# LiZhuoHong/SegLand

Measured on AMD Instinct MI355X. Metric: 512x512 tiles/sec fwd+bwd PSPNet-POP, higher is better.
Workload: dtype bf16; 1 GPU; PSPNet-POP resnet50 bf16, batch 16/GPU, 512x512, 8 logit channels, train_base.py loop body (fwd+loss+bwd+clip+AdamW x2), 1 x MI355X; global_batch=16, parallelism=dp1

## Files before the change

### segland_amd/csrc/ppm.hip

```cpp
#include "common.h"

namespace {

struct PpmGeom {
  int B, H, W, C, nlevels;
  int sizes[4];
  int rowoff[5];
  int ncy, ncx;
  int yb[40], xb[40];
};

inline int bin_start(int i, int in, int out) { return (i * in) / out; }
inline int bin_end(int i, int in, int out) { return ((i + 1) * in + out - 1) / out; }
__device__ __forceinline__ int d_bin_start(int i, int in, int out) { return (i * in) / out; }
__device__ __forceinline__ int d_bin_end(int i, int in, int out) { return ((i + 1) * in + out - 1) / out; }

int make_bounds(const SlPpmDesc* d, int in, int* out) {
  bool mark[4097] = {false};
  if (in > 4096) return -1;
  for (int l = 0; l < d->nlevels; ++l)
    for (int i = 0; i < d->sizes[l]; ++i) { mark[bin_start(i, in, d->sizes[l])] = true; mark[bin_end(i, in, d->sizes[l])] = true; }
  int n = 0;
  for (int v = 0; v <= in; ++v) if (mark[v]) { if (n >= 40) return -1; out[n++] = v; }
  return n - 1;
}

int make_geom(const SlPpmDesc* d, PpmGeom& g) {
  SL_REQUIRE(d && d->B > 0 && d->H > 0 && d->W > 0 && d->C > 0 && d->C % 8 == 0, "ppm: bad sizes");
  SL_REQUIRE(d->nlevels >= 1 && d->nlevels <= 4, "ppm: 1..4 levels");
  g.B = d->B; g.H = d->H; g.W = d->W; g.C = d->C; g.nlevels = d->nlevels;
  int off = 0;
  for (int l = 0; l < 4; ++l) {
    g.sizes[l] = l < d->nlevels ? d->sizes[l] : 0;
    g.rowoff[l] = off;
    if (l < d->nlevels) { SL_REQUIRE(d->sizes[l] >= 1 && d->sizes[l] <= 64, "ppm: bad level size"); off += d->B * d->sizes[l] * d->sizes[l]; }
  }
  g.rowoff[4] = off;
  g.ncy = make_bounds(d, d->H, g.yb);
  g.ncx = make_bounds(d, d->W, g.xb);
  SL_REQUIRE(g.ncy > 0 && g.ncx > 0, "ppm: too many distinct bin boundaries");
  return 0;
}

template <typename T>
__global__ void ppm_cells_kernel(PpmGeom g, const T* __restrict__ x, float* __restrict__ cells) {
  constexpr int V = Vec16<T>::N;
  const int nv = g.C / V;
  const long long total = (long long)g.B * g.ncy * g.ncx * nv;
  for (long long i = blockIdx.x * (long long)blockDim.x + threadIdx.x; i < total; i += (long long)gridDim.x * blockDim.x) {
    const int v = (int)(i % nv); long long r = i / nv;
    const int cx = (int)(r % g.ncx); r /= g.ncx;
    const int cy = (int)(r % g.ncy); const int b = (int)(r / g.ncy);
    float s[V];
#pragma unroll
    for (int k = 0; k < V; ++k) s[k] = 0.f;
    for (int y = g.yb[cy]; y < g.yb[cy + 1]; ++y)
      for (int xx = g.xb[cx]; xx < g.xb[cx + 1]; ++xx) {
        float t[V];
        unpack16<T>(*(const uint4*)(x + ((size_t)(b * g.H + y) * g.W + xx) * g.C + v * V), t);
#pragma unroll
        for (int k = 0; k < V; ++k) s[k] += t[k];
      }
    float* o = cells + (size_t)i * V;
#pragma unroll
    for (int k = 0; k < V; ++k) o[k] = s[k];
  }
}

template <typename T>
__global__ __launch_bounds__(256) void ppm_cells_rows_kernel(PpmGeom g, const T* __restrict__ x, float* __restrict__ cells) {
  constexpr int V = Vec16<T>::N;
  __shared__ float red[8][32][V + 1];
  const int nv = g.C / V, vblocks = (nv + 31) / 32;
  int bid = blockIdx.x;
  const int vb = bid % vblocks; bid /= vblocks;
  const int cx = bid % g.ncx; bid /= g.ncx;
  const int cy = bid % g.ncy; const int b = bid / g.ncy;
  const int lv = threadIdx.x & 31, rl = threadIdx.x >> 5;
  const int v = vb * 32 + lv;
  float s[V];
#pragma unroll
  for (int k = 0; k < V; ++k) s[k] = 0.f;
  if (v < nv)
    for (int y = g.yb[cy] + rl; y < g.yb[cy + 1]; y += 8)
      for (int xx = g.xb[cx]; xx < g.xb[cx + 1]; ++xx) {
        float t[V];
        unpack16<T>(*(const uint4*)(x + ((size_t)(b * g.H + y) * g.W + xx) * g.C + v * V), t);
#pragma unroll
        for (int k = 0; k < V; ++k) s[k] += t[k];
      }
#pragma unroll
  for (int k = 0; k < V; ++k) red[rl][lv][k] = s[k];
  __syncthreads();
  if (rl == 0 && v < nv) {
    float* o = cells + ((((size_t)b * g.ncy + cy) * g.ncx + cx) * nv + v) * V;
#pragma unroll
    for (int k = 0; k < V; ++k) {
      float a = red[0][lv][k];
#pragma unroll
      for (int r = 1; r < 8; ++r) a += red[r][lv][k];
      o[k] = a;
    }
  }
}

__global__ void ppm_bins_kernel(PpmGeom g, const float* __restrict__ cells, float* __restrict__ pooled) {
  const long long total = (long long)g.rowoff[4] * g.C;
  for (long long i = blockIdx.x * (long long)blockDim.x + threadIdx.x; i < total; i += (long long)gridDim.x * blockDim.x) {
    const int c = (int)(i % g.C); const int row = (int)(i / g.C);
    int l = 0;
    while (l + 1 < g.nlevels && row >= g.rowoff[l + 1]) ++l;
    const int s = g.sizes[l];
    int r = row - g.rowoff[l];
    const int j = r % s; r /= s;
    const int ii = r % s; const int b = r / s;
    const int ys = d_bin_start(ii, g.H, s), ye = d_bin_end(ii, g.H, s), xs = d_bin_start(j, g.W, s), xe = d_bin_end(j, g.W, s);
    float sum = 0.f;
    for (int cy = 0; cy < g.ncy; ++cy) {
      if (g.yb[cy] < ys || g.yb[cy + 1] > ye) continue;
      for (int cx = 0; cx < g.ncx; ++cx) {
        if (g.xb[cx] < xs || g.xb[cx + 1] > xe) continue;
        sum += cells[(((size_t)b * g.ncy + cy) * g.ncx + cx) * g.C + c];
      }
    }
    pooled[i] = sum / (float)((ye - ys) * (xe - xs));
  }
}

__global__ void ppm_pool_bwd_cells_kernel(PpmGeom g, const float* __restrict__ dpooled, float* __restrict__ gcell) {
  const long long total = (long long)g.B * g.ncy * g.ncx * g.C;
  for (long long i = blockIdx.x * (long long)blockDim.x + threadIdx.x; i < total; i += (long long)gridDim.x * blockDim.x) {
    const int c = (int)(i % g.C); long long r = i / g.C;
    const int cx = (int)(r % g.ncx); r /= g.ncx;
    const int cy = (int)(r % g.ncy); const int b = (int)(r / g.ncy);
    const int y0 = g.yb[cy], y1 = g.yb[cy + 1], x0 = g.xb[cx], x1 = g.xb[cx + 1];
    float acc = 0.f;
    int nbins = 0;
    for (int l = 0; l < g.nlevels; ++l) nbins += g.sizes[l] * g.sizes[l];
    if (g.C % 64 == 0 && nbins <= 64) {
      const int lane = threadIdx.x & 63;
      float wq = 0.f; int rowq = 0;
      {
        int q = lane, l = 0;
        while (l < g.nlevels && q >= g.sizes[l] * g.sizes[l]) { q -= g.sizes[l] * g.sizes[l]; ++l; }
        if (l < g.nlevels) {
          const int s = g.sizes[l], ii = q / s, j = q - ii * s;
          const int ys = d_bin_start(ii, g.H, s), ye = d_bin_end(ii, g.H, s), xs = d_bin_start(j, g.W, s), xe = d_bin_end(j, g.W, s);
          if (!(y0 < ys || y1 > ye) && !(x0 < xs || x1 > xe)) { wq = 1.f / (float)((ye - ys) * (xe - xs)); rowq = g.rowoff[l] + (b * s + ii) * s + j; }
        }
      }
      for (int q = 0; q < nbins; ++q) {
        const float w = __shfl(wq, q, 64);
        if (w == 0.f) continue;
        acc += dpooled[(size_t)__shfl(rowq, q, 64) * g.C + c] * w;
      }
      gcell[i] = acc;
      continue;
    }
    for (int l = 0; l < g.nlevels; ++l) {
      const int s = g.sizes[l];
      for (int ii = 0; ii < s; ++ii) {
        const int ys = d_bin_start(ii, g.H, s), ye = d_bin_end(ii, g.H, s);
        if (y0 < ys || y1 > ye) continue;
        for (int j = 0; j < s; ++j) {
          const int xs = d_bin_start(j, g.W, s), xe = d_bin_end(j, g.W, s);
          if (x0 < xs || x1 > xe) continue;
          acc += dpooled[((size_t)g.rowoff[l] + (size_t)(b * s + ii) * s + j) * g.C + c] * (1.f / (float)((ye - ys) * (xe - xs)));
        }
      }
    }
    gcell[i] = acc;
  }
}

template <typename T>
__global__ __launch_bounds__(256) void ppm_pool_bwd_kernel(PpmGeom g, const float* __restrict__ gcell, const T* __restrict__ dcat, int cat_pitch, int cat_off,
                                                           T* __restrict__ dx) {
  constexpr int V = Vec16<T>::N;
  __shared__ int cxs[4096];
  const int by = blockIdx.x, b = by / g.H, y = by - b * g.H;
  int cy = 0;
  while (cy + 1 < g.ncy && y >= g.yb[cy + 1]) ++cy;
  for (int xx = threadIdx.x; xx < g.W; xx += 256) {
    int cx = 0;
    while (cx + 1 < g.ncx && xx >= g.xb[cx + 1]) ++cx;
    cxs[xx] = cx;
  }
  __syncthreads();
  const int nv = g.C / V;
  const float* gc = gcell + ((size_t)b * g.ncy + cy) * g.ncx * g.C;
  const size_t row = (size_t)by * g.W;
  for (int i = threadIdx.x; i < g.W * nv; i += 256) {
    const int xx = i / nv, v = i - xx * nv;
    float acc[V];
    if (dcat) unpack16<T>(*(const uint4*)(dcat + (row + xx) * cat_pitch + cat_off + v * V), acc);
    else {
#pragma unroll
      for (int k = 0; k < V; ++k) acc[k] = 0.f;
    }
    const float* t = gc + (size_t)cxs[xx] * g.C + v * V;
#pragma unroll
    for (int k = 0; k < V; k += 4) {
      const float4 q = *(const float4*)(t + k);
      acc[k] += q.x; acc[k + 1] += q.y; acc[k + 2] += q.z; acc[k + 3] += q.w;
    }
    *(uint4*)(dx + ((row + xx) * nv + v) * V) = pack16<T>(acc);
  }
}

__device__ __forceinline__ void src_index_ac0(int dst, int in, int out, int& i0, int& i1, float& l1) {
  const float scale = (float)in / (float)out;
  float src = scale * ((float)dst + 0.5f) - 0.5f;
  if (src < 0.f) src = 0.f;
  i0 = (int)src;
  i1 = i0 + (i0 < in - 1 ? 1 : 0);
  l1 = src - (float)i0;
  l1 = l1 < 0.f ? 0.f : (l1 > 1.f ? 1.f : l1);
}

template <typename T>
__global__ void ppm_upsample_fwd_kernel(PpmGeom g, int Cs, const float* __restrict__ stage, T* __restrict__ priors) {
  constexpr int V = Vec16<T>::N;
  const int nv = Cs / V, pitch = g.nlevels * Cs;
  const long long total = (long long)g.B * g.H * g.W * g.nlevels * nv;
  for (long long i = blockIdx.x * (long long)blockDim.x + threadIdx.x; i < total; i += (long long)gridDim.x * blockDim.x) {
    const int v = (int)(i % nv); long long r = i / nv;
    const int l = (int)(r % g.nlevels); r /= g.nlevels;
    const int xx = (int)(r % g.W); r /= g.W;
    const int y = (int)(r % g.H); const int b = (int)(r / g.H);
// ... 369 lines not shown
    SL_TRY(sl_launch("ppm_cells_rows_kernel", ppm_cells_rows_kernel<bf16_t>, dim3((unsigned)(g.B * g.ncy * g.ncx * ((g.C / 8 + 31) / 32))), dim3(256), 0, st, g, (const bf16_t*)x, cells));
  else
    SL_TRY(sl_by_dtype(d->dtype, "ppm_pool_fwd", [&](auto t) -> int {
      using T = decltype(t);
      return sl_launch("ppm_cells_kernel", ppm_cells_kernel<T>, dim3(gs_blocks((long long)g.B * g.ncy * g.ncx * g.C / Vec16<T>::N)), dim3(256), 0, st, g, (const T*)x, cells);
    }));
  return sl_launch("ppm_bins_kernel", ppm_bins_kernel, dim3(gs_blocks((long long)g.rowoff[4] * g.C)), dim3(256), 0, st, g, cells, pooled);
}

extern "C" int sl_ppm_pool_bwd(const SlPpmDesc* d, const float* dpooled, const void* dcat, int cat_pitch, int cat_off, void* dx,
                               void* workspace, size_t workspace_bytes, sl_stream_t stream) {
  PpmGeom g;
  if (int e = make_geom(d, g)) return e;
  SL_REQUIRE(dpooled && dx && workspace, "ppm_pool_bwd: null buffer");
  SL_REQUIRE(!dcat || (cat_pitch >= cat_off + g.C && cat_pitch % 8 == 0 && cat_off % 8 == 0), "ppm_pool_bwd: bad concat geometry");
  SL_REQUIRE(g.W <= 4096, "ppm_pool_bwd: W > 4096");
  const size_t need = (size_t)g.B * g.ncy * g.ncx * g.C * sizeof(float);
  if (workspace_bytes < need) { sl_set_error("ppm_pool_bwd: workspace %zu < %zu", workspace_bytes, need); return SL_EWORKSPACE; }
  hipStream_t st = (hipStream_t)stream;
  float* gcell = (float*)workspace;
  return sl_by_dtype(d->dtype, "ppm_pool_bwd", [&](auto t) -> int {
    using T = decltype(t);
    SL_TRY(sl_launch("ppm_pool_bwd_cells_kernel", ppm_pool_bwd_cells_kernel, dim3(gs_blocks((long long)g.B * g.ncy * g.ncx * g.C)), dim3(256), 0, st, g, dpooled, gcell));
    return sl_launch("ppm_pool_bwd_kernel", ppm_pool_bwd_kernel<T>, dim3(g.B * g.H), dim3(256), 0, st, g, gcell, (const T*)dcat, cat_pitch, cat_off, (T*)dx);
  });
}

extern "C" int sl_ppm_upsample_fwd(const SlPpmDesc* d, int Cs, const float* stage, void* priors, sl_stream_t stream) {
  PpmGeom g;
  if (int e = make_geom(d, g)) return e;
  SL_REQUIRE(stage && priors && Cs > 0 && Cs % 8 == 0, "ppm_upsample_fwd: bad args");
  return sl_by_dtype(d->dtype, "ppm_upsample_fwd", [&](auto t) -> int {
    using T = decltype(t);
    return sl_launch("ppm_upsample_fwd_kernel", ppm_upsample_fwd_kernel<T>, dim3(gs_blocks((long long)g.B * g.H * g.W * g.nlevels * Cs / Vec16<T>::N)), dim3(256), 0, (hipStream_t)stream, g, Cs, stage, (T*)priors);
  });
}

extern "C" int sl_ppm_upsample_bwd(const SlPpmDesc* d, int Cs, const void* dcat, int cat_pitch, float* dstage, void* workspace,
                                   size_t workspace_bytes, sl_stream_t stream) {
  PpmGeom g;
  if (int e = make_geom(d, g)) return e;
  SL_REQUIRE(dcat && dstage && workspace && Cs > 0 && Cs % 8 == 0 && cat_pitch >= g.nlevels * Cs, "ppm_upsample_bwd: bad args");
  const int nlj = sum_sizes(g);
  const size_t need = (size_t)g.B * g.H * nlj * Cs * sizeof(float);
  if (workspace_bytes < need) { sl_set_error("ppm_upsample_bwd: workspace %zu < %zu", workspace_bytes, need); return SL_EWORKSPACE; }
  hipStream_t st = (hipStream_t)stream;
  float* tmp = (float*)workspace;
// ... 339 lines not shown
```

### segland_amd/csrc/stem.hip

```cpp
#include "common.h"

namespace {

constexpr int TS = 16;
constexpr int PS = (TS - 1) * 2 + 7;
constexpr int NTAP = 147;

__device__ __forceinline__ void load_patch(float* patch, const float* img, int b, int H, int W, int oy0, int ox0, int tid) {
  for (int e = tid; e < 3 * PS * PS; e += 256) {
    const int c = e / (PS * PS), r = (e / PS) % PS, q = e % PS;
    const int iy = 2 * oy0 - 3 + r, ix = 2 * ox0 - 3 + q;
    float v = 0.f;
    if ((unsigned)iy < (unsigned)H && (unsigned)ix < (unsigned)W) v = img[((size_t)(b * 3 + c) * H + iy) * W + ix];
    patch[e] = v;
  }
}

template <typename T>
__global__ __launch_bounds__(256) void stem_conv_fwd_kernel(const float* __restrict__ img, const float* __restrict__ w,
                                                            T* __restrict__ y, float* __restrict__ part, int B, int H, int W) {
  extern __shared__ __attribute__((aligned(16))) float sm[];
  float* wl = sm;
  float* patch = sm + NTAP * 64;
  const int Ho = H / 2, Wo = W / 2;
// ... 54 lines not shown
      for (int k = 0; k < 16; ++k) {
        part[((size_t)blockIdx.x * 2 + 0) * 64 + cg * 16 + k] = s1[k];
        part[((size_t)blockIdx.x * 2 + 1) * 64 + cg * 16 + k] = s2[k];
      }
    }
  }
}

constexpr int MP = 38;
constexpr int KSTEPS = 10;

__global__ void stem_weight_frag_kernel(const float* __restrict__ w, uint4* __restrict__ wfrag) {
  const int t = blockIdx.x * blockDim.x + threadIdx.x;
  if (t >= 2 * KSTEPS * 64) return;
  const int lane = t & 63, ks = (t >> 6) % KSTEPS, nb = (t >> 6) / KSTEPS;
  const int n = nb * 32 + (lane & 31), k0 = ks * 16 + (lane >> 5) * 8;
  unsigned short v[8];
#pragma unroll
  for (int e = 0; e < 8; ++e) v[e] = k0 + e < NTAP ? from_f<bf16_t>(w[n * NTAP + k0 + e]) : (unsigned short)0;
  wfrag[t] = make_uint4(v[0] | ((unsigned)v[1] << 16), v[2] | ((unsigned)v[3] << 16), v[4] | ((unsigned)v[5] << 16), v[6] | ((unsigned)v[7] << 16));
}

__host__ __device__ constexpr int stem_tap_off(int k) { return k < NTAP ? ((k / 49) * PS + (k % 49) / 7) * MP + (k % 7) : 0; }

template <int KS>
__device__ __forceinline__ void stem_kstep(const bf16_t* __restrict__ patch, const int (&pbase)[2], int fh, const uint4* __restrict__ wfrag, int lane, f32x16_t (&acc)[2][2]) {
  const uint4 w0 = wfrag[(0 * KSTEPS + KS) * 64 + lane], w1 = wfrag[(1 * KSTEPS + KS) * 64 + lane];
  int off[8];
#pragma unroll
  for (int e = 0; e < 8; ++e) off[e] = fh ? stem_tap_off(KS * 16 + 8 + e) : stem_tap_off(KS * 16 + e);
#pragma unroll
  for (int rb = 0; rb < 2; ++rb) {
    unsigned v[8];
#pragma unroll
    for (int e = 0; e < 8; ++e) v[e] = patch[pbase[rb] + off[e]];
    const uint4 a = make_uint4(v[0] | (v[1] << 16), v[2] | (v[3] << 16), v[4] | (v[5] << 16), v[6] | (v[7] << 16));
    acc[rb][0] = __builtin_amdgcn_mfma_f32_32x32x16_bf16(__builtin_bit_cast(bf16x8_t, w0), __builtin_bit_cast(bf16x8_t, a), acc[rb][0], 0, 0, 0);
    acc[rb][1] = __builtin_amdgcn_mfma_f32_32x32x16_bf16(__builtin_bit_cast(bf16x8_t, w1), __builtin_bit_cast(bf16x8_t, a), acc[rb][1], 0, 0, 0);
  }
}

__global__ __launch_bounds__(256) void stem_conv_fwd_mfma_kernel(const float* __restrict__ img, const uint4* __restrict__ wfrag,
                                                                 bf16_t* __restrict__ y, float* __restrict__ part, int B, int H, int W) {
  extern __shared__ __attribute__((aligned(16))) unsigned char smem[];
  bf16_t* patch = (bf16_t*)smem;
  bf16_t* outt = (bf16_t*)smem;
  float* red = (float*)(smem + 256 * 72 * sizeof(bf16_t));
  const int Ho = H / 2, Wo = W / 2;
  const int tx = cdiv(Wo, TS), ty = cdiv(Ho, TS);
  const int tid = threadIdx.x, lane = tid & 63, wave = tid >> 6;
  int blk = blockIdx.x;
  const int bx = blk % tx; blk /= tx;
  const int by = blk % ty; const int b = blk / ty;
  {
    const int rr = tid >> 1, half = tid & 1;
    if (rr < 3 * PS) {
      const int c = rr / PS, r = rr - c * PS;
      const int iy = 2 * by * TS - 3 + r, ix0 = 2 * bx * TS - 3;
      const bool rowok = (unsigned)iy < (unsigned)H;
      const float* src = img + ((size_t)(b * 3 + c) * H + (rowok ? iy : 0)) * W;
      bf16_t* dst = patch + rr * MP;
      const int q0 = half * 19, q1 = half ? PS : 19;
      for (int q = q0; q < q1; ++q) {
        const int ix = ix0 + q;
        dst[q] = from_f<bf16_t>(rowok && (unsigned)ix < (unsigned)W ? src[ix] : 0.f);
      }
    }
  }
  __syncthreads();

  const int l31 = lane & 31, fh = lane >> 5;
  f32x16_t acc[2][2];
#pragma unroll
  for (int rb = 0; rb < 2; ++rb)
#pragma unroll
    for (int nb = 0; nb < 2; ++nb)
#pragma unroll
      for (int r = 0; r < 16; ++r) acc[rb][nb][r] = 0.f;
  int pbase[2];
#pragma unroll
  for (int rb = 0; rb < 2; ++rb) {
    const int pidx = wave * 64 + rb * 32 + l31;
    pbase[rb] = (2 * (pidx >> 4)) * MP + 2 * (pidx & 15);
  }
  stem_kstep<0>(patch, pbase, fh, wfrag, lane, acc); stem_kstep<1>(patch, pbase, fh, wfrag, lane, acc);
  stem_kstep<2>(patch, pbase, fh, wfrag, lane, acc); stem_kstep<3>(patch, pbase, fh, wfrag, lane, acc);
  stem_kstep<4>(patch, pbase, fh, wfrag, lane, acc); stem_kstep<5>(patch, pbase, fh, wfrag, lane, acc);
  stem_kstep<6>(patch, pbase, fh, wfrag, lane, acc); stem_kstep<7>(patch, pbase, fh, wfrag, lane, acc);
  stem_kstep<8>(patch, pbase, fh, wfrag, lane, acc); stem_kstep<9>(patch, pbase, fh, wfrag, lane, acc);
  __syncthreads();
#pragma unroll
// ... 10 lines not shown
      }
  }
  __syncthreads();
  for (int e = tid; e < 256 * 8; e += 256) {
    const int pidx = e >> 3, ch8 = e & 7;
    const int oy = by * TS + (pidx >> 4), ox = bx * TS + (pidx & 15);
    if (oy < Ho && ox < Wo) *(uint4*)(y + ((size_t)(b * Ho + oy) * Wo + ox) * 64 + ch8 * 8) = *(const uint4*)(outt + pidx * 72 + ch8 * 8);
  }
  if (part) {
    const int ch = tid & 63, qtr = tid >> 6;
    float a = 0.f, c = 0.f;
    for (int pp = 0; pp < 64; ++pp) {
      const int pidx = qtr * 64 + pp;
      const int oy = by * TS + (pidx >> 4), ox = bx * TS + (pidx & 15);
      if (oy < Ho && ox < Wo) { const float v = to_f<bf16_t>(outt[pidx * 72 + ch]); a += v; c += v * v; }
    }
    red[(qtr * 2 + 0) * 64 + ch] = a; red[(qtr * 2 + 1) * 64 + ch] = c;
    __syncthreads();
    if (tid < 128) {
      const int which = tid >> 6;
      part[((size_t)blockIdx.x * 2 + which) * 64 + ch] = red[(0 * 2 + which) * 64 + ch] + red[(1 * 2 + which) * 64 + ch] + red[(2 * 2 + which) * 64 + ch] + red[(3 * 2 + which) * 64 + ch];
    }
  }
}

template <typename T, int CH>
__global__ void stem_bn_relu_pool_fwd_kernel(const T* __restrict__ c0, const float* __restrict__ scale, const float* __restrict__ shift,
                                             T* __restrict__ pooled, uint8_t* __restrict__ idx, int B, int Hc, int Wc, int Cr) {
  constexpr int V = Vec16<T>::N;
  const int Cn = CH ? CH : Cr, NV = Cn / V;
  const int Hp = (Hc + 1) / 2, Wp = (Wc + 1) / 2;
  const long long total = (long long)B * Hp * Wp * NV;
  for (long long i = blockIdx.x * (long long)blockDim.x + threadIdx.x; i < total; i += (long long)gridDim.x * blockDim.x) {
    const int v = (int)(i % NV); long long r = i / NV;
    const int px = (int)(r % Wp); r /= Wp;
    const int py = (int)(r % Hp); const int b = (int)(r / Hp);
    float best[V]; int bi[V];
#pragma unroll
    for (int k = 0; k < V; ++k) { best[k] = -INFINITY; bi[k] = 0; }
    float sc[V], sh[V];
#pragma unroll
    for (int k = 0; k < V; ++k) { sc[k] = scale[v * V + k]; sh[k] = shift[v * V + k]; }
    for (int ky = 0; ky < 3; ++ky) {
      const int yy = 2 * py - 1 + ky;
      if ((unsigned)yy >= (unsigned)Hc) continue;
      for (int kx = 0; kx < 3; ++kx) {
// ... 6 lines not shown
          float a = xv[k] * sc[k] + sh[k];
          a = a > 0.f ? a : 0.f;
          if (a > best[k] || a != a) { best[k] = a; bi[k] = ky * 3 + kx; }
        }
      }
    }
    const size_t o = ((size_t)(b * Hp + py) * Wp + px) * Cn + v * V;
    *(uint4*)(pooled + o) = pack16<T>(best);
    if (idx) {
#pragma unroll
      for (int k = 0; k < V; ++k) idx[o + k] = (uint8_t)bi[k];
    }
  }
}

template <typename T, bool STAT, int CH>
__global__ __launch_bounds__(256) void stem_pool_relu_bwd_kernel(const T* __restrict__ dp, const uint8_t* __restrict__ idx, const T* __restrict__ c0,
                                          const float* __restrict__ scale, const float* __restrict__ shift, T* __restrict__ g0,
                                          int B, int Hc, int Wc, const float* __restrict__ mean, const float* __restrict__ invstd, float* __restrict__ part, int Cr) {
  constexpr int V = Vec16<T>::N;
  const int Cn = CH ? CH : Cr, NV = Cn / V;
  const int Hp = (Hc + 1) / 2, Wp = (Wc + 1) / 2;
  const long long total = (long long)B * Hc * Wc * NV;
  float s1[V], s2[V], mu[V], is[V];
  if (STAT) {
    const int v0 = threadIdx.x % NV;
#pragma unroll
    for (int k = 0; k < V; ++k) { s1[k] = 0.f; s2[k] = 0.f; mu[k] = mean[v0 * V + k]; is[k] = invstd[v0 * V + k]; }
  }
  for (long long i = blockIdx.x * (long long)blockDim.x + threadIdx.x; i < total; i += (long long)gridDim.x * blockDim.x) {
    const int v = (int)(i % NV); long long r = i / NV;
    const int x = (int)(r % Wc); r /= Wc;
    const int y = (int)(r % Hc); const int b = (int)(r / Hc);
    float g[V], xv[V];
#pragma unroll
    for (int k = 0; k < V; ++k) g[k] = 0.f;
    const int py_lo = y / 2, py_hi = (y + 1) / 2, px_lo = x / 2, px_hi = (x + 1) / 2;
    for (int py = py_lo; py <= py_hi; ++py) {
      if (py >= Hp) continue;
      const int ky = y - (2 * py - 1);
      for (int px = px_lo; px <= px_hi; ++px) {
        if (px >= Wp) continue;
        const int kx = x - (2 * px - 1);
        const size_t o = ((size_t)(b * Hp + py) * Wp + px) * Cn + v * V;
        float d[V];
        unpack16<T>(*(const uint4*)(dp + o), d);
        const int want = ky * 3 + kx;
#pragma unroll
        for (int k = 0; k < V; ++k) if (idx[o + k] == want) g[k] += d[k];
      }
    }
    const size_t oc = ((size_t)(b * Hc + y) * Wc + x) * Cn + v * V;
    unpack16<T>(*(const uint4*)(c0 + oc), xv);
#pragma unroll
    for (int k = 0; k < V; ++k) g[k] = (xv[k] * scale[v * V + k] + shift[v * V + k]) > 0.f ? g[k] : 0.f;
    const uint4 q = pack16<T>(g);
    *(uint4*)(g0 + oc) = q;
    if (STAT) {
      float gr[V];
      unpack16<T>(q, gr);
#pragma unroll
      for (int k = 0; k < V; ++k) { s1[k] += gr[k]; s2[k] += gr[k] * ((xv[k] - mu[k]) * is[k]); }
    }
  }
  if (STAT) {
    __shared__ float red[256 * 2 * V];
#pragma unroll
    for (int k = 0; k < V; ++k) { red[threadIdx.x * 2 * V + k] = s1[k]; red[threadIdx.x * 2 * V + V + k] = s2[k]; }
    __syncthreads();
    const int nthr = CH ? 256 : (int)blockDim.x;
    for (int e = threadIdx.x; e < 2 * Cn; e += nthr) {
      const int which = e / Cn, c = e - which * Cn, v = c / V, k = c % V;
      float a = 0.f;
      for (int j = 0; j < nthr / NV; ++j) a += red[(j * NV + v) * 2 * V + which * V + k];
      part[((size_t)blockIdx.x * 2 + which) * Cn + c] = a;
    }
  }
}

template <typename T>
__global__ __launch_bounds__(256) void stem_wgrad_kernel(const float* __restrict__ img, const T* __restrict__ dc0, float* __restrict__ ws,
                                                         int B, int H, int W, int tiles_per_blk, int ntiles) {
  extern __shared__ __attribute__((aligned(16))) float sm[];
  float* dyl = sm;
  float* patch = sm + 256 * 64;
  const int Ho = H / 2, Wo = W / 2;
  const int tx = cdiv(Wo, TS), ty = cdiv(Ho, TS);
  const int tid = threadIdx.x, n = tid & 63;
  const int g = __builtin_amdgcn_readfirstlane(tid >> 6);
  float acc[6][7];
#pragma unroll
  for (int i = 0; i < 6; ++i)
#pragma unroll
    for (int k = 0; k < 7; ++k) acc[i][k] = 0.f;
  for (int t = 0; t < tiles_per_blk; ++t) {
    int tile = blockIdx.x * tiles_per_blk + t;
    if (tile >= ntiles) break;
// ... 15 lines not shown
#pragma unroll
      for (int i = 0; i < 6; ++i) {
        const int id = g + 4 * i;
        if (id < 21) {
          const int c = id / 7, ky = id - 7 * c;
          const float* prow = patch + (c * PS + 2 * py + ky) * PS + 2 * px;
#pragma unroll
          for (int k = 0; k < 7; ++k) acc[i][k] = fmaf(a, prow[k], acc[i][k]);
        }
      }
    }
  }
  float* o = ws + (size_t)blockIdx.x * 64 * NTAP + n * NTAP;
#pragma unroll
  for (int i = 0; i < 6; ++i) {
    const int id = g + 4 * i;
    if (id < 21) {
#pragma unroll
      for (int k = 0; k < 7; ++k) o[id * 7 + k] = acc[i][k];
    }
  }
}

__global__ __launch_bounds__(256) void stem_wgrad_mfma_kernel(const float* __restrict__ img, const bf16_t* __restrict__ dc0, float* __restrict__ ws,
                                                              int B, int H, int W, int ntiles) {
  extern __shared__ __attribute__((aligned(16))) unsigned char smem[];
  bf16_t* patch = (bf16_t*)smem;
  bf16_t* dct = patch + 3 * PS * MP + 6;
  float* red = (float*)smem;
  const int Ho = H / 2, Wo = W / 2;
  const int tx = cdiv(Wo, TS), ty = cdiv(Ho, TS);
  const int tid = threadIdx.x, lane = tid & 63, wave = tid >> 6, l31 = lane & 31, fh = lane >> 5;
  f32x16_t acc[2][5];
#pragma unroll
  for (int nb = 0; nb < 2; ++nb)
#pragma unroll
    for (int kb = 0; kb < 5; ++kb)
#pragma unroll
      for (int r = 0; r < 16; ++r) acc[nb][kb][r] = 0.f;
  int toff[5];
#pragma unroll
  for (int kb = 0; kb < 5; ++kb) {
    const int k = kb * 32 + l31;
    const int c = k / 49, r = k - c * 49, ky = r / 7, kx = r - ky * 7;
    toff[kb] = k < NTAP ? (c * PS + ky) * MP + kx : 0;
  }
  for (int tile = blockIdx.x; tile < ntiles; tile += gridDim.x) {
    int blk = tile;
    const int bx = blk % tx; blk /= tx;
    const int by = blk % ty; const int b = blk / ty;
    {
      const int rr = tid >> 1, half = tid & 1;
      if (rr < 3 * PS) {
        const int c = rr / PS, r = rr - c * PS;
        const int iy = 2 * by * TS - 3 + r, ix0 = 2 * bx * TS - 3;
        const bool rowok = (unsigned)iy < (unsigned)H;
        const float* src = img + ((size_t)(b * 3 + c) * H + (rowok ? iy : 0)) * W;
        bf16_t* dst = patch + rr * MP;
        const int q0 = half * 19, q1 = half ? PS : 19;
        for (int q = q0; q < q1; ++q) {
          const int ix = ix0 + q;
          dst[q] = from_f<bf16_t>(rowok && (unsigned)ix < (unsigned)W ? src[ix] : 0.f);
        }
      }
    }
    for (int e = tid; e < 256 * 8; e += 256) {
      const int pidx = e >> 3, ch8 = e & 7;
      const int oy = by * TS + (pidx >> 4), ox = bx * TS + (pidx & 15);
      uint4 v = make_uint4(0, 0, 0, 0);
      if (oy < Ho && ox < Wo) v = *(const uint4*)(dc0 + ((size_t)(b * Ho + oy) * Wo + ox) * 64 + ch8 * 8);
      *(uint4*)(dct + pidx * 72 + ch8 * 8) = v;
    }
    __syncthreads();
#pragma unroll
    for (int ks = 0; ks < 4; ++ks) {
      const int prow = wave * 64 + ks * 16 + fh * 8;
      uint4 fa[2];
#pragma unroll
      for (int nb = 0; nb < 2; ++nb) {
        unsigned v[8];
#pragma unroll
        for (int e = 0; e < 8; ++e) v[e] = dct[(prow + e) * 72 + nb * 32 + l31];
        fa[nb] = make_uint4(v[0] | (v[1] << 16), v[2] | (v[3] << 16), v[4] | (v[5] << 16), v[6] | (v[7] << 16));
      }
      const int pb = (2 * (wave * 4 + ks)) * MP + 2 * (fh * 8);
#pragma unroll
      for (int kb = 0; kb < 5; ++kb) {
        unsigned v[8];
#pragma unroll
        for (int e = 0; e < 8; ++e) v[e] = patch[pb + toff[kb] + 2 * e];
        const uint4 fb = make_uint4(v[0] | (v[1] << 16), v[2] | (v[3] << 16), v[4] | (v[5] << 16), v[6] | (v[7] << 16));
#pragma unroll
        for (int nb = 0; nb < 2; ++nb)
          acc[nb][kb] = __builtin_amdgcn_mfma_f32_32x32x16_bf16(__builtin_bit_cast(bf16x8_t, fa[nb]), __builtin_bit_cast(bf16x8_t, fb), acc[nb][kb], 0, 0, 0);
      }
    }
    __syncthreads();
  }
  float* out = ws + (size_t)blockIdx.x * 64 * NTAP;
#pragma unroll
  for (int nb = 0; nb < 2; ++nb)
#pragma unroll
    for (int kb = 0; kb < 5; ++kb) {
#pragma unroll
      for (int r = 0; r < 16; ++r) red[(wave * 16 + r) * 64 + lane] = acc[nb][kb][r];
      __syncthreads();
      for (int e = tid; e < 16 * 64; e += 256) {
        const int r = e >> 6, ln = e & 63;
        const float t = red[(0 * 16 + r) * 64 + ln] + red[(1 * 16 + r) * 64 + ln] + red[(2 * 16 + r) * 64 + ln] + red[(3 * 16 + r) * 64 + ln];
        const int n = nb * 32 + (r & 3) + 8 * (r >> 2) + 4 * (ln >> 5), k = kb * 32 + (ln & 31);
        if (k < NTAP) out[n * NTAP + k] = t;
      }
      __syncthreads();
    }
// ... 113 lines not shown
}

extern "C" int sl_stem_pool_relu_bwd_bnstat_c_rows(int B, int Hc, int Wc, int C) { return pool_bwd_stat_rows(B, Hc, Wc, C); }
extern "C" int sl_stem_pool_relu_bwd_bnstat_c(int dtype, const void* dpooled, const uint8_t* argmax, const void* c0, const float* scale, const float* shift,
                                              const float* mean, const float* invstd, void* g0, float* stat_partial, int B, int Hc, int Wc, int C, sl_stream_t stream) {
  SL_REQUIRE(dpooled && argmax && c0 && scale && shift && mean && invstd && g0 && stat_partial && B > 0 && Hc > 0 && Wc > 0, "stem_pool_relu_bwd_bnstat_c: bad args");
  SL_REQUIRE(pool_c_ok(C), "stem_pool_relu_bwd_bnstat_c: C = %d is not a multiple of 64 in 64..1024", C);
  SL_REQUIRE(dtype == SL_BF16 || dtype == SL_F32, "stem_pool_relu_bwd_bnstat_c: bad dtype");
  SL_REQUIRE((long long)B * Hc * Wc * C < (1ll << 31), "stem_pool_relu_bwd_bnstat_c: more than 2^31 elements");
  return launch_pool_bwd("stem_pool_relu_bwd_bnstat_c", dtype, pool_bwd_stat_rows(B, Hc, Wc, C), pool_bwd_threads(dtype, C), dpooled, argmax, c0, scale, shift, g0, B, Hc, Wc, C, mean, invstd, stat_partial, stream);
}

extern "C" size_t sl_stem_conv_bwd_weight_workspace(int B, int H, int W) {
  return (size_t)stem_wgrad_blocks(stem_tiles(B, H, W)) * 64 * NTAP * sizeof(float);
}

extern "C" int sl_stem_conv_bwd_weight(int dtype, const float* img_nchw, const void* dc0, float* dw_oihw, void* workspace,
                                       size_t workspace_bytes, int B, int H, int W, sl_stream_t stream) {
  SL_REQUIRE(img_nchw && dc0 && dw_oihw && workspace && B > 0 && H % 2 == 0 && W % 2 == 0, "stem_conv_bwd_weight: bad args");
  const int ntiles = stem_tiles(B, H, W), nblk = stem_wgrad_blocks(ntiles), tpb = cdiv(ntiles, nblk);
  if (workspace_bytes < (size_t)nblk * 64 * NTAP * sizeof(float)) { sl_set_error("stem_conv_bwd_weight: workspace too small"); return SL_EWORKSPACE; }
  hipStream_t st = (hipStream_t)stream;
  if (dtype == SL_BF16) {
    const size_t l2 = (size_t)(3 * PS * MP + 6) * sizeof(bf16_t) + 256 * 72 * sizeof(bf16_t);
    SL_TRY(sl_launch("stem_wgrad_mfma_kernel", stem_wgrad_mfma_kernel, dim3(nblk), dim3(256), l2, st, img_nchw, (const bf16_t*)dc0, (float*)workspace, B, H, W, ntiles));
  } else if (dtype == SL_F32) {
    const size_t lds = (256 * 64 + 3 * PS * PS) * sizeof(float);
    SL_TRY(sl_launch("stem_wgrad_kernel", stem_wgrad_kernel<float>, dim3(nblk), dim3(256), lds, st, img_nchw, (const float*)dc0, (float*)workspace, B, H, W, tpb, ntiles));
  } else SL_REQUIRE(false, "stem_conv_bwd_weight: bad dtype");
  return sl_colsum_finalize((const float*)workspace, nblk, 64 * NTAP, dw_oihw, stream);
}

extern "C" int sl_stem_im2col(int dtype, const float* img_nchw, void* col, int B, int H, int W, sl_stream_t stream) {
  SL_REQUIRE(img_nchw && col && B > 0 && H % 2 == 0 && W % 2 == 0, "stem_im2col: bad args");
  const long long total = (long long)B * (H / 2) * (W / 2) * (dtype == SL_BF16 ? 24 : 48);
  const int blocks = (int)((total + 255) / 256 < 32768 ? (total + 255) / 256 : 32768);
  return sl_by_dtype(dtype, "stem_im2col", [&](auto t) -> int {
    using T = decltype(t);
    return sl_launch("stem_im2col_kernel", stem_im2col_kernel<T>, dim3(blocks), dim3(256), 0, (hipStream_t)stream, img_nchw, (T*)col, B, H, W);
  });
}
```

Measured before the change: 722.9 tiles/s.

## Batch loads in PPM kernels and repack stem patches for paired LDS reads

The PPM cell and bin reductions are rewritten as flat loops that issue eight loads before accumulating. The pooling backward now walks only the active bins via a ballot mask, and the per-row scatter kernel is split into width segments with a u8 lookup table and four-way load batching. In the stem kernels, the input patch is stored as odd/even planes so that MFMA fragments can be built from 32-bit LDS reads instead of per-element 16-bit gathers. The maxpool-ReLU backward gains hoisted scale/shift values, incremental index stepping and packed argmax loads. These changes aim to cut memory latency stalls and LDS instruction count, at the cost of more complex indexing and a larger LDS footprint in the wgrad kernel.

```diff
diff --git a/segland_amd/csrc/ppm.hip b/segland_amd/csrc/ppm.hip
--- a/segland_amd/csrc/ppm.hip
+++ b/segland_amd/csrc/ppm.hip
@@ -44,7 +44,7 @@
 
 template <typename T>
 __global__ void ppm_cells_kernel(PpmGeom g, const T* __restrict__ x, float* __restrict__ cells) {
-  constexpr int V = Vec16<T>::N;
+  constexpr int V = Vec16<T>::N, U = 8;
   const int nv = g.C / V;
   const long long total = (long long)g.B * g.ncy * g.ncx * nv;
   for (long long i = blockIdx.x * (long long)blockDim.x + threadIdx.x; i < total; i += (long long)gridDim.x * blockDim.x) {
@@ -54,13 +54,28 @@
     float s[V];
 #pragma unroll
     for (int k = 0; k < V; ++k) s[k] = 0.f;
-    for (int y = g.yb[cy]; y < g.yb[cy + 1]; ++y)
-      for (int xx = g.xb[cx]; xx < g.xb[cx + 1]; ++xx) {
-        float t[V];
-        unpack16<T>(*(const uint4*)(x + ((size_t)(b * g.H + y) * g.W + xx) * g.C + v * V), t);
-#pragma unroll
-        for (int k = 0; k < V; ++k) s[k] += t[k];
-      }
+    const int y0 = g.yb[cy], x0 = g.xb[cx], w = g.xb[cx + 1] - x0, n = (g.yb[cy + 1] - y0) * w;
+    const T* px = x + ((size_t)(b * g.H + y0) * g.W + x0) * g.C + v * V;
+    const size_t next_row = (size_t)(g.W - w) * g.C;
+    int col = 0;
+    for (int j = 0; j < n; j += U) {
+      uint4 q[U];
+#pragma unroll
+      for (int u = 0; u < U; ++u)
+        if (j + u < n) {
+          q[u] = *(const uint4*)px;
+          px += g.C;
+          if (++col == w) { col = 0; px += next_row; }
+        }
+#pragma unroll
+      for (int u = 0; u < U; ++u)
+        if (j + u < n) {
+          float t[V];
+          unpack16<T>(q[u], t);
+#pragma unroll
+          for (int k = 0; k < V; ++k) s[k] += t[k];
+        }
+    }
     float* o = cells + (size_t)i * V;
 #pragma unroll
     for (int k = 0; k < V; ++k) o[k] = s[k];
@@ -105,6 +120,7 @@
 }
 
 __global__ void ppm_bins_kernel(PpmGeom g, const float* __restrict__ cells, float* __restrict__ pooled) {
+  constexpr int U = 8;
   const long long total = (long long)g.rowoff[4] * g.C;
   for (long long i = blockIdx.x * (long long)blockDim.x + threadIdx.x; i < total; i += (long long)gridDim.x * blockDim.x) {
     const int c = (int)(i % g.C); const int row = (int)(i / g.C);
@@ -115,13 +131,28 @@
     const int j = r % s; r /= s;
     const int ii = r % s; const int b = r / s;
     const int ys = d_bin_start(ii, g.H, s), ye = d_bin_end(ii, g.H, s), xs = d_bin_start(j, g.W, s), xe = d_bin_end(j, g.W, s);
+    int cya = 0, cyb = g.ncy, cxa = 0, cxb = g.ncx;
+    while (cya < g.ncy && g.yb[cya] < ys) ++cya;
+    while (cyb > cya && g.yb[cyb] > ye) --cyb;
+    while (cxa < g.ncx && g.xb[cxa] < xs) ++cxa;
+    while (cxb > cxa && g.xb[cxb] > xe) --cxb;
+    const int w = cxb - cxa, n = (cyb - cya) * w;
+    const float* p = cells + (((size_t)b * g.ncy + cya) * g.ncx + cxa) * g.C + c;
+    const size_t next_row = (size_t)(g.ncx - w) * g.C;
     float sum = 0.f;
-    for (int cy = 0; cy < g.ncy; ++cy) {
-      if (g.yb[cy] < ys || g.yb[cy + 1] > ye) continue;
-      for (int cx = 0; cx < g.ncx; ++cx) {
-        if (g.xb[cx] < xs || g.xb[cx + 1] > xe) continue;
-        sum += cells[(((size_t)b * g.ncy + cy) * g.ncx + cx) * g.C + c];
-      }
+    int col = 0;
+    for (int e = 0; e < n; e += U) {
+      float q[U];
+#pragma unroll
+      for (int u = 0; u < U; ++u)
+        if (e + u < n) {
+          q[u] = *p;
+          p += g.C;
+          if (++col == w) { col = 0; p += next_row; }
+        }
+#pragma unroll
+      for (int u = 0; u < U; ++u)
+        if (e + u < n) sum += q[u];
     }
     pooled[i] = sum / (float)((ye - ys) * (xe - xs));
   }
@@ -149,10 +180,21 @@
           if (!(y0 < ys || y1 > ye) && !(x0 < xs || x1 > xe)) { wq = 1.f / (float)((ye - ys) * (xe - xs)); rowq = g.rowoff[l] + (b * s + ii) * s + j; }
         }
       }
-      for (int q = 0; q < nbins; ++q) {
-        const float w = __shfl(wq, q, 64);
-        if (w == 0.f) continue;
-        acc += dpooled[(size_t)__shfl(rowq, q, 64) * g.C + c] * w;
+      unsigned long long m = __ballot(wq != 0.f);
+      while (m) {
+        float w[4], d[4]; int rw[4];
+#pragma unroll
+        for (int u = 0; u < 4; ++u) {
+          const int q = m ? __ffsll((long long)m) - 1 : 0;
+          w[u] = __shfl(wq, q, 64); rw[u] = __shfl(rowq, q, 64);
+          if (!m) { w[u] = 0.f; rw[u] = 0; }
+          m &= m - 1;
+        }
+#pragma unroll
+        for (int u = 0; u < 4; ++u) d[u] = dpooled[(size_t)rw[u] * g.C + c];
+#pragma unroll
+        for (int u = 0; u < 4; ++u)
+          if (w[u] != 0.f) acc += d[u] * w[u];
       }
       gcell[i] = acc;
       continue;
@@ -173,38 +215,51 @@
   }
 }
 
-template <typename T>
+constexpr int PBW_SEG = 4096;
+template <typename T, bool P2>
 __global__ __launch_bounds__(256) void ppm_pool_bwd_kernel(PpmGeom g, const float* __restrict__ gcell, const T* __restrict__ dcat, int cat_pitch, int cat_off,
-                                                           T* __restrict__ dx) {
+                                                           T* __restrict__ dx, int nseg, int nvsh) {
   constexpr int V = Vec16<T>::N;
-  __shared__ int cxs[4096];
-  const int by = blockIdx.x, b = by / g.H, y = by - b * g.H;
+  __shared__ uint8_t cxs[PBW_SEG];
+  const int nv = g.C / V;
+  const int by = blockIdx.x / nseg, seg = blockIdx.x - by * nseg, b = by / g.H, y = by - b * g.H;
+  const int i_lo = seg * PBW_SEG, i_hi = i_lo + PBW_SEG < g.W * nv ? i_lo + PBW_SEG : g.W * nv;
+  const int xa = i_lo / nv, xe = (i_hi - 1) / nv;
   int cy = 0;
   while (cy + 1 < g.ncy && y >= g.yb[cy + 1]) ++cy;
-  for (int xx = threadIdx.x; xx < g.W; xx += 256) {
+  for (int xx = xa + threadIdx.x; xx <= xe; xx += 256) {
     int cx = 0;
     while (cx + 1 < g.ncx && xx >= g.xb[cx + 1]) ++cx;
-    cxs[xx] = cx;
+    cxs[xx - xa] = (uint8_t)cx;
   }
   __syncthreads();
-  const int nv = g.C / V;
   const float* gc = gcell + ((size_t)b * g.ncy + cy) * g.ncx * g.C;
   const size_t row = (size_t)by * g.W;
-  for (int i = threadIdx.x; i < g.W * nv; i += 256) {
-    const int xx = i / nv, v = i - xx * nv;
-    float acc[V];
-    if (dcat) unpack16<T>(*(const uint4*)(dcat + (row + xx) * cat_pitch + cat_off + v * V), acc);
-    else {
-#pragma unroll
-      for (int k = 0; k < V; ++k) acc[k] = 0.f;
-    }
-    const float* t = gc + (size_t)cxs[xx] * g.C + v * V;
-#pragma unroll
-    for (int k = 0; k < V; k += 4) {
-      const float4 q = *(const float4*)(t + k);
-      acc[k] += q.x; acc[k + 1] += q.y; acc[k + 2] += q.z; acc[k + 3] += q.w;
-    }
-    *(uint4*)(dx + ((row + xx) * nv + v) * V) = pack16<T>(acc);
+  for (int i0 = i_lo + threadIdx.x; i0 < i_hi; i0 += 1024) {
+    uint4 d[4];
+    float4 q[4][V / 4];
+    size_t o[4];
+#pragma unroll
+    for (int u = 0; u < 4; ++u) {
+      const int i = i0 + u * 256;
+      if (i < i_hi) {
+        const int xx = P2 ? i >> nvsh : i / nv, v = i - xx * nv;
+        d[u] = dcat ? *(const uint4*)(dcat + (row + xx) * cat_pitch + cat_off + v * V) : make_uint4(0u, 0u, 0u, 0u);
+        const float* t = gc + (size_t)cxs[xx - xa] * g.C + v * V;
+#pragma unroll
+        for (int k = 0; k < V / 4; ++k) q[u][k] = *(const float4*)(t + 4 * k);
+        o[u] = ((row + xx) * nv + v) * V;
+      }
+    }
+#pragma unroll
+    for (int u = 0; u < 4; ++u) {
+      if (i0 + u * 256 >= i_hi) break;
+      float acc[V];
+      unpack16<T>(d[u], acc);
+#pragma unroll
+      for (int k = 0; k < V / 4; ++k) { acc[4 * k] += q[u][k].x; acc[4 * k + 1] += q[u][k].y; acc[4 * k + 2] += q[u][k].z; acc[4 * k + 3] += q[u][k].w; }
+      *(uint4*)(dx + o[u]) = pack16<T>(acc);
+    }
   }
 }
 
@@ -620,7 +675,10 @@
   return sl_by_dtype(d->dtype, "ppm_pool_bwd", [&](auto t) -> int {
     using T = decltype(t);
     SL_TRY(sl_launch("ppm_pool_bwd_cells_kernel", ppm_pool_bwd_cells_kernel, dim3(gs_blocks((long long)g.B * g.ncy * g.ncx * g.C)), dim3(256), 0, st, g, dpooled, gcell));
-    return sl_launch("ppm_pool_bwd_kernel", ppm_pool_bwd_kernel<T>, dim3(g.B * g.H), dim3(256), 0, st, g, gcell, (const T*)dcat, cat_pitch, cat_off, (T*)dx);
+    const int nv = g.C / Vec16<T>::N, nseg = cdiv((long long)g.W * nv, PBW_SEG);
+    const bool p2 = (nv & (nv - 1)) == 0;
+    return sl_launch("ppm_pool_bwd_kernel", p2 ? ppm_pool_bwd_kernel<T, true> : ppm_pool_bwd_kernel<T, false>, dim3((unsigned)(g.B * g.H * nseg)), dim3(256), 0, st, g, gcell, (const T*)dcat, cat_pitch,
+                     cat_off, (T*)dx, nseg, __builtin_ctz((unsigned)nv));
   });
 }
 
diff --git a/segland_amd/csrc/stem.hip b/segland_amd/csrc/stem.hip
--- a/segland_amd/csrc/stem.hip
+++ b/segland_amd/csrc/stem.hip
@@ -100,21 +100,54 @@
 }
 
 __host__ __device__ constexpr int stem_tap_off(int k) { return k < NTAP ? ((k / 49) * PS + (k % 49) / 7) * MP + (k % 7) : 0; }
+constexpr int PATCH2 = 3 * PS * MP;
+__host__ __device__ constexpr int stem_pair_lo(int t) { return (stem_tap_off(t) & 1) ? PATCH2 + stem_tap_off(t) - 1 : stem_tap_off(t); }
+__host__ __device__ constexpr bool stem_pair_split(int t) { return t < NTAP && t % 7 == 6; }
+__host__ __device__ constexpr int stem_pair_hi(int t) { return stem_pair_split(t) ? stem_tap_off(t + 1) : 0; }
 
 template <int KS>
 __device__ __forceinline__ void stem_kstep(const bf16_t* __restrict__ patch, const int (&pbase)[2], int fh, const uint4* __restrict__ wfrag, int lane, f32x16_t (&acc)[2][2]) {
   const uint4 w0 = wfrag[(0 * KSTEPS + KS) * 64 + lane], w1 = wfrag[(1 * KSTEPS + KS) * 64 + lane];
-  int off[8];
-#pragma unroll
-  for (int e = 0; e < 8; ++e) off[e] = fh ? stem_tap_off(KS * 16 + 8 + e) : stem_tap_off(KS * 16 + e);
 #pragma unroll
   for (int rb = 0; rb < 2; ++rb) {
-    unsigned v[8];
-#pragma unroll
-    for (int e = 0; e < 8; ++e) v[e] = patch[pbase[rb] + off[e]];
-    const uint4 a = make_uint4(v[0] | (v[1] << 16), v[2] | (v[3] << 16), v[4] | (v[5] << 16), v[6] | (v[7] << 16));
+    unsigned v[4];
+#pragma unroll
+    for (int j = 0; j < 4; ++j) {
+      const int t0 = KS * 16 + 2 * j, t1 = t0 + 8;
+      unsigned d = *(const unsigned*)(patch + pbase[rb] + (fh ? stem_pair_lo(t1) : stem_pair_lo(t0)));
+      if (stem_pair_split(t0) || stem_pair_split(t1)) {
+        const unsigned hi = patch[pbase[rb] + (fh ? stem_pair_hi(t1) : stem_pair_hi(t0))];
+        if (fh ? stem_pair_split(t1) : stem_pair_split(t0)) d = (d & 0xffffu) | (hi << 16);
+      }
+      v[j] = d;
+    }
+    const uint4 a = make_uint4(v[0], v[1], v[2], v[3]);
     acc[rb][0] = __builtin_amdgcn_mfma_f32_32x32x16_bf16(__builtin_bit_cast(bf16x8_t, w0), __builtin_bit_cast(bf16x8_t, a), acc[rb][0], 0, 0, 0);
     acc[rb][1] = __builtin_amdgcn_mfma_f32_32x32x16_bf16(__builtin_bit_cast(bf16x8_t, w1), __builtin_bit_cast(bf16x8_t, a), acc[rb][1], 0, 0, 0);
+  }
+}
+
+__device__ __forceinline__ void stem_fill_pairs(bf16_t* __restrict__ dst, int pitch, int step, const float* __restrict__ img, int b, int H, int W, int iy0, int ix0, int wave, int lane) {
+  typedef __attribute__((ext_vector_type(2))) __bf16 bf16x2_t;
+  typedef __attribute__((ext_vector_type(2))) float f32x2_t;
+  const int ix = ix0 + lane, ixn = ix + step;
+  const bool ok0 = lane < PS && (unsigned)ix < (unsigned)W, ok1 = lane + step < PS && (unsigned)ixn < (unsigned)W;
+  const int xa = ix < 0 ? 0 : (ix < W ? ix : W - 1), xb = ixn < 0 ? 0 : (ixn < W ? ixn : W - 1);
+  for (int r0 = wave; r0 < 3 * PS; r0 += 28) {
+    float va[7], vb[7];
+#pragma unroll
+    for (int u = 0; u < 7; ++u) {
+      const int rr = r0 + 4 * u < 3 * PS ? r0 + 4 * u : 3 * PS - 1;
+      const int c = rr / PS, iy = iy0 + rr - c * PS;
+      const bool rowok = (unsigned)iy < (unsigned)H;
+      const float* src = img + ((size_t)(b * 3 + c) * H + (rowok ? iy : 0)) * W;
+      const float a = src[xa], bb = src[xb];
+      va[u] = rowok && ok0 ? a : 0.f; vb[u] = rowok && ok1 ? bb : 0.f;
+    }
+#pragma unroll
+    for (int u = 0; u < 7; ++u)
+      if (r0 + 4 * u < 3 * PS && lane < PS)
+        *(unsigned*)(dst + (r0 + 4 * u) * pitch) = __builtin_bit_cast(unsigned, __builtin_convertvector((f32x2_t){va[u], vb[u]}, bf16x2_t));
   }
 }
 
@@ -130,21 +163,7 @@
   int blk = blockIdx.x;
   const int bx = blk % tx; blk /= tx;
   const int by = blk % ty; const int b = blk / ty;
-  {
-    const int rr = tid >> 1, half = tid & 1;
-    if (rr < 3 * PS) {
-      const int c = rr / PS, r = rr - c * PS;
-      const int iy = 2 * by * TS - 3 + r, ix0 = 2 * bx * TS - 3;
-      const bool rowok = (unsigned)iy < (unsigned)H;
-      const float* src = img + ((size_t)(b * 3 + c) * H + (rowok ? iy : 0)) * W;
-      bf16_t* dst = patch + rr * MP;
-      const int q0 = half * 19, q1 = half ? PS : 19;
-      for (int q = q0; q < q1; ++q) {
-        const int ix = ix0 + q;
-        dst[q] = from_f<bf16_t>(rowok && (unsigned)ix < (unsigned)W ? src[ix] : 0.f);
-      }
-    }
-  }
+  stem_fill_pairs(patch + ((lane & 1) ? PATCH2 + lane - 1 : lane), MP, 1, img, b, H, W, 2 * by * TS - 3, 2 * bx * TS - 3, wave, lane);
   __syncthreads();
 
   const int l31 = lane & 31, fh = lane >> 5;
@@ -201,6 +220,17 @@
       part[((size_t)blockIdx.x * 2 + which) * 64 + ch] = red[(0 * 2 + which) * 64 + ch] + red[(1 * 2 + which) * 64 + ch] + red[(2 * 2 + which) * 64 + ch] + red[(3 * 2 + which) * 64 + ch];
     }
   }
+}
+
+template <int V> __device__ __forceinline__ unsigned long long load_pos(const uint8_t* p, bool aligned) {
+  if (aligned) {
+    if constexpr (V == 8) { const uint2 q = *(const uint2*)p; return ((unsigned long long)q.y << 32) | q.x; }
+    else return *(const unsigned*)p;
+  }
+  unsigned long long r = 0;
+#pragma unroll
+  for (int k = 0; k < V; ++k) r |= (unsigned long long)p[k] << (8 * k);
+  return r;
 }
 
 template <typename T, int CH>
@@ -253,38 +283,55 @@
   const int Cn = CH ? CH : Cr, NV = Cn / V;
   const int Hp = (Hc + 1) / 2, Wp = (Wc + 1) / 2;
   const long long total = (long long)B * Hc * Wc * NV;
-  float s1[V], s2[V], mu[V], is[V];
+  const bool pos_aligned = ((size_t)idx & (V - 1)) == 0;
+  const int v = threadIdx.x % NV;
+  float s1[V], s2[V], mu[V], is[V], sc[V], sh[V];
+#pragma unroll
+  for (int k = 0; k < V; ++k) { sc[k] = scale[v * V + k]; sh[k] = shift[v * V + k]; }
   if (STAT) {
-    const int v0 = threadIdx.x % NV;
-#pragma unroll
-    for (int k = 0; k < V; ++k) { s1[k] = 0.f; s2[k] = 0.f; mu[k] = mean[v0 * V + k]; is[k] = invstd[v0 * V + k]; }
-  }
-  for (long long i = blockIdx.x * (long long)blockDim.x + threadIdx.x; i < total; i += (long long)gridDim.x * blockDim.x) {
-    const int v = (int)(i % NV); long long r = i / NV;
-    const int x = (int)(r % Wc); r /= Wc;
-    const int y = (int)(r % Hc); const int b = (int)(r / Hc);
+#pragma unroll
+    for (int k = 0; k < V; ++k) { s1[k] = 0.f; s2[k] = 0.f; mu[k] = mean[v * V + k]; is[k] = invstd[v * V + k]; }
+  }
+  const long long istep = (long long)gridDim.x * blockDim.x;
+  long long i = blockIdx.x * (long long)blockDim.x + threadIdx.x;
+  long long r = i / NV;
+  int x = (int)(r % Wc); r /= Wc;
+  int y = (int)(r % Hc); int b = (int)(r / Hc);
+  r = istep / NV;
+  const int dx = (int)(r % Wc); r /= Wc;
+  const int dy = (int)(r % Hc); const int db = (int)(r / Hc);
+  for (; i < total; i += istep) {
+    const int py_lo = y / 2, px_lo = x / 2;
+    const int ny = 1 + ((y & 1) && py_lo + 1 < Hp), nx = 1 + ((x & 1) && px_lo + 1 < Wp);
+    uint4 dq[4]; unsigned long long pq[4];
+#pragma unroll
+    for (int u = 0; u < 4; ++u) {
+      const int wy = u >> 1, wx = u & 1;
+      if (wy < ny && wx < nx) {
+        const size_t o = ((size_t)(b * Hp + py_lo + wy) * Wp + px_lo + wx) * Cn + v * V;
+        dq[u] = *(const uint4*)(dp + o);
+        pq[u] = load_pos<V>(idx + o, pos_aligned);
+      }
+    }
+    const size_t oc = ((size_t)(b * Hc + y) * Wc + x) * Cn + v * V;
+    const uint4 cq = *(const uint4*)(c0 + oc);
     float g[V], xv[V];
 #pragma unroll
     for (int k = 0; k < V; ++k) g[k] = 0.f;
-    const int py_lo = y / 2, py_hi = (y + 1) / 2, px_lo = x / 2, px_hi = (x + 1) / 2;
-    for (int py = py_lo; py <= py_hi; ++py) {
-      if (py >= Hp) continue;
-      const int ky = y - (2 * py - 1);
-      for (int px = px_lo; px <= px_hi; ++px) {
-        if (px >= Wp) continue;
-        const int kx = x - (2 * px - 1);
-        const size_t o = ((size_t)(b * Hp + py) * Wp + px) * Cn + v * V;
+#pragma unroll
+    for (int u = 0; u < 4; ++u) {
+      const int wy = u >> 1, wx = u & 1;
+      if (wy < ny && wx < nx) {
+        const unsigned want = (unsigned)((y - (2 * (py_lo + wy) - 1)) * 3 + (x - (2 * (px_lo + wx) - 1)));
         float d[V];
-        unpack16<T>(*(const uint4*)(dp + o), d);
-        const int want = ky * 3 + kx;
-#pragma unroll
-        for (int k = 0; k < V; ++k) if (idx[o + k] == want) g[k] += d[k];
-      }
-    }
-    const size_t oc = ((size_t)(b * Hc + y) * Wc + x) * Cn + v * V;
-    unpack16<T>(*(const uint4*)(c0 + oc), xv);
-#pragma unroll
-    for (int k = 0; k < V; ++k) g[k] = (xv[k] * scale[v * V + k] + shift[v * V + k]) > 0.f ? g[k] : 0.f;
+        unpack16<T>(dq[u], d);
+#pragma unroll
+        for (int k = 0; k < V; ++k) if (((unsigned)(pq[u] >> (8 * k)) & 0xffu) == want) g[k] += d[k];
+      }
+    }
+    unpack16<T>(cq, xv);
+#pragma unroll
+    for (int k = 0; k < V; ++k) g[k] = (xv[k] * sc[k] + sh[k]) > 0.f ? g[k] : 0.f;
     const uint4 q = pack16<T>(g);
     *(uint4*)(g0 + oc) = q;
     if (STAT) {
@@ -293,6 +340,9 @@
 #pragma unroll
       for (int k = 0; k < V; ++k) { s1[k] += gr[k]; s2[k] += gr[k] * ((xv[k] - mu[k]) * is[k]); }
     }
+    x += dx; if (x >= Wc) { x -= Wc; ++y; }
+    y += dy; if (y >= Hc) { y -= Hc; ++b; }
+    b += db;
   }
   if (STAT) {
     __shared__ float red[256 * 2 * V];
@@ -301,9 +351,9 @@
     __syncthreads();
     const int nthr = CH ? 256 : (int)blockDim.x;
     for (int e = threadIdx.x; e < 2 * Cn; e += nthr) {
-      const int which = e / Cn, c = e - which * Cn, v = c / V, k = c % V;
+      const int which = e / Cn, c = e - which * Cn, cv = c / V, k = c % V;
       float a = 0.f;
-      for (int j = 0; j < nthr / NV; ++j) a += red[(j * NV + v) * 2 * V + which * V + k];
+      for (int j = 0; j < nthr / NV; ++j) a += red[(j * NV + cv) * 2 * V + which * V + k];
       part[((size_t)blockIdx.x * 2 + which) * Cn + c] = a;
     }
   }
@@ -365,11 +415,13 @@
   }
 }
 
+constexpr int WP = 20;
+constexpr int WPLANE = 3 * PS * WP;
 __global__ __launch_bounds__(256) void stem_wgrad_mfma_kernel(const float* __restrict__ img, const bf16_t* __restrict__ dc0, float* __restrict__ ws,
                                                               int B, int H, int W, int ntiles) {
   extern __shared__ __attribute__((aligned(16))) unsigned char smem[];
   bf16_t* patch = (bf16_t*)smem;
-  bf16_t* dct = patch + 3 * PS * MP + 6;
+  bf16_t* dct = patch + 4 * WPLANE;
   float* red = (float*)smem;
   const int Ho = H / 2, Wo = W / 2;
   const int tx = cdiv(Wo, TS), ty = cdiv(Ho, TS);
@@ -386,27 +438,15 @@
   for (int kb = 0; kb < 5; ++kb) {
     const int k = kb * 32 + l31;
     const int c = k / 49, r = k - c * 49, ky = r / 7, kx = r - ky * 7;
-    toff[kb] = k < NTAP ? (c * PS + ky) * MP + kx : 0;
-  }
+    const int j = kx >> 1;
+    toff[kb] = k < NTAP ? (2 * (kx & 1) + (j & 1)) * WPLANE + (c * PS + ky) * WP + j - (j & 1) : 0;
+  }
+  bf16_t* const fill_dst = patch + (2 * (lane & 1) + ((lane >> 1) & 1)) * WPLANE + (lane >> 1) - ((lane >> 1) & 1);
   for (int tile = blockIdx.x; tile < ntiles; tile += gridDim.x) {
     int blk = tile;
     const int bx = blk % tx; blk /= tx;
     const int by = blk % ty; const int b = blk / ty;
-    {
-      const int rr = tid >> 1, half = tid & 1;
-      if (rr < 3 * PS) {
-        const int c = rr / PS, r = rr - c * PS;
-        const int iy = 2 * by * TS - 3 + r, ix0 = 2 * bx * TS - 3;
-        const bool rowok = (unsigned)iy < (unsigned)H;
-        const float* src = img + ((size_t)(b * 3 + c) * H + (rowok ? iy : 0)) * W;
-        bf16_t* dst = patch + rr * MP;
-        const int q0 = half * 19, q1 = half ? PS : 19;
-        for (int q = q0; q < q1; ++q) {
-          const int ix = ix0 + q;
-          dst[q] = from_f<bf16_t>(rowok && (unsigned)ix < (unsigned)W ? src[ix] : 0.f);
-        }
-      }
-    }
+    stem_fill_pairs(fill_dst, WP, 2, img, b, H, W, 2 * by * TS - 3, 2 * bx * TS - 3, wave, lane);
     for (int e = tid; e < 256 * 8; e += 256) {
       const int pidx = e >> 3, ch8 = e & 7;
       const int oy = by * TS + (pidx >> 4), ox = bx * TS + (pidx & 15);
@@ -426,13 +466,11 @@
         for (int e = 0; e < 8; ++e) v[e] = dct[(prow + e) * 72 + nb * 32 + l31];
         fa[nb] = make_uint4(v[0] | (v[1] << 16), v[2] | (v[3] << 16), v[4] | (v[5] << 16), v[6] | (v[7] << 16));
       }
-      const int pb = (2 * (wave * 4 + ks)) * MP + 2 * (fh * 8);
+      const int pb = (2 * (wave * 4 + ks)) * WP + fh * 8;
 #pragma unroll
       for (int kb = 0; kb < 5; ++kb) {
-        unsigned v[8];
-#pragma unroll
-        for (int e = 0; e < 8; ++e) v[e] = patch[pb + toff[kb] + 2 * e];
-        const uint4 fb = make_uint4(v[0] | (v[1] << 16), v[2] | (v[3] << 16), v[4] | (v[5] << 16), v[6] | (v[7] << 16));
+        const unsigned* pv = (const unsigned*)(patch + pb + toff[kb]);
+        const uint4 fb = make_uint4(pv[0], pv[1], pv[2], pv[3]);
 #pragma unroll
         for (int nb = 0; nb < 2; ++nb)
           acc[nb][kb] = __builtin_amdgcn_mfma_f32_32x32x16_bf16(__builtin_bit_cast(bf16x8_t, fa[nb]), __builtin_bit_cast(bf16x8_t, fb), acc[nb][kb], 0, 0, 0);
@@ -592,7 +630,7 @@
   if (workspace_bytes < (size_t)nblk * 64 * NTAP * sizeof(float)) { sl_set_error("stem_conv_bwd_weight: workspace too small"); return SL_EWORKSPACE; }
   hipStream_t st = (hipStream_t)stream;
   if (dtype == SL_BF16) {
-    const size_t l2 = (size_t)(3 * PS * MP + 6) * sizeof(bf16_t) + 256 * 72 * sizeof(bf16_t);
+    const size_t l2 = (size_t)4 * WPLANE * sizeof(bf16_t) + 256 * 72 * sizeof(bf16_t);
     SL_TRY(sl_launch("stem_wgrad_mfma_kernel", stem_wgrad_mfma_kernel, dim3(nblk), dim3(256), l2, st, img_nchw, (const bf16_t*)dc0, (float*)workspace, B, H, W, ntiles));
   } else if (dtype == SL_F32) {
     const size_t lds = (256 * 64 + 3 * PS * PS) * sizeof(float);
```

Measured after the change: 726.3 tiles/s, median of 6. No clear change (+0.5%).
